# matthewscottgordon/vanrijn

Hardware: AMD Instinct MI355X
Metric: Msamples/s + achieved HBM GB/s, 1024x1024 bunny @256spp, 1/2/4/8 GPUs (higher is better)
Workload: dtype f64; 1 GPU; main.rs scene (plane, 3 spheres, Lambertian bunny), 1024x1024 @256spp per frame split over 1 GPU(s) (256 each); config=c3, width=1024, height=1024, spp_per_gpu=256, triangles=69312, bvh_depth=20, parallelism=spp-split x1, RCCL reduce, streams=1, pmc_key=main 1024x1024 spp256

## Files before the change

include/vanrijn_amd.h:

```cpp
#ifndef VANRIJN_AMD_H
#define VANRIJN_AMD_H

#include <stddef.h>
#include <stdint.h>

#ifdef __cplusplus
extern "C" {
#endif

#define VR_ABI_VERSION 10
#define VR_HAS_FILM 1
#define VR_HAS_ONE_BVH 1
#define VR_MAX_SPECTRUM_SAMPLES 64
#define VR_RECURSION_LIMIT 128

typedef enum vr_status {
    VR_OK = 0,
    VR_ERROR_INVALID_ARGUMENT = -1,
    VR_ERROR_OUT_OF_MEMORY = -2,
    VR_ERROR_DEVICE = -3,
    VR_ERROR_NO_DEVICE = -4,
    VR_ERROR_SINGULAR_BASIS = -5,
    VR_ERROR_IO = -6,
    VR_ERROR_UNSUPPORTED = -7,
// ... 339 lines not shown
void vr_colour_xyz_for_wavelength(double wavelength, double out[3]);
int vr_load_obj(const char* path, uint64_t* triangle_count, double** vertices, double** normals);
void vr_mesh_free(double* vertices, double* normals);
int vr_load_obj_groups(const char* path, uint64_t* triangle_count, double** vertices, double** normals,
                       uint32_t** group, uint32_t* group_count, char** names);
void vr_obj_groups_free(uint32_t* group, char* names);

int vr_tone_map_device(const double* state, uint64_t pixel_count, uint8_t* rgb_out, int device, void* stream);
int vr_tone_map(const double* colour_xyz, uint64_t pixel_count, uint8_t* rgb_out, int device);
int vr_write_png(const char* path, const uint8_t* rgb, uint32_t width, uint32_t height);

int vr_scene_set_staging_limit(vr_scene* scene, uint64_t bytes);

int vr_debug_set_fault_object(vr_scene* scene, int32_t object);

int vr_debug_set_launch_flags(vr_scene* scene, uint32_t flags);
int vr_scene_needs_wide_offsets(uint64_t triangle_count, uint64_t wide_node_count);
#define VR_CHOICE_COUNTING 1u
#define VR_CHOICE_RECORD 2u
#define VR_CHOICE_WHITTED 4u
#define VR_CHOICE_COOP_GATED 8u
#define VR_CHOICE_WIDE_OFFSETS 16u
#define VR_CHOICE_MULTI_BVH 32u
int vr_launch_takes_one_bvh(uint64_t bvh_count, int32_t root4, uint32_t other, int32_t stack_depth, int32_t stack16);
int vr_scene_launch_variant(const vr_scene* scene, uint64_t pixel_samples, uint32_t launch_flags, int32_t recording,
                            uint32_t* variant);

int vr_device_count(void);
const char* vr_last_error(void);
uint32_t vr_abi_version(void);

#ifdef __cplusplus
}
#endif
#endif
```

vanrijn_amd/_native.py:

```python
import ctypes as C
import os

HERE = os.path.dirname(os.path.abspath(__file__))
LIB_PATH = os.environ.get("VR_LIBRARY") or os.path.join(HERE, "lib", "libvanrijn_amd.so")

VR_OK = 0
STATUS = {
    0: "VR_OK", -1: "VR_ERROR_INVALID_ARGUMENT", -2: "VR_ERROR_OUT_OF_MEMORY", -3: "VR_ERROR_DEVICE",
    -4: "VR_ERROR_NO_DEVICE", -5: "VR_ERROR_SINGULAR_BASIS", -6: "VR_ERROR_IO", -7: "VR_ERROR_UNSUPPORTED",
    -8: "VR_ERROR_HOST_ONLY",
}
MATERIAL_LAMBERTIAN, MATERIAL_REFLECTIVE, MATERIAL_PHONG, MATERIAL_DIELECTRIC = 0, 1, 2, 3
PRIMITIVE_PLANE, PRIMITIVE_SPHERE = 0, 1
OBJECT_PRIMITIVE_LIST, OBJECT_BVH = 0, 1
SCENE_HOST_ONLY = 1
SCENE_DEVICE_BVH = 2
SCENE_REFERENCE_BVH = 4
SCENE_DEVICE_SAH = 8
SCENE_GREEDY_COLLAPSE = 16
SCENE_WIDE_OFFSETS = 32
LAUNCH_TIMED, LAUNCH_COUNTERS, LAUNCH_DEFER_TIMES, LAUNCH_NO_CULL = 1, 2, 4, 8
LAUNCH_NO_DIST_CULL, LAUNCH_NO_COOP, LAUNCH_NO_LONE_WALK, LAUNCH_STACK32, LAUNCH_MULTI_BVH = 16, 32, 64, 128, 256
VARIANT_COOP, VARIANT_WIDE_OFFSETS, VARIANT_STACK16, VARIANT_ONE_BVH = 1, 2, 4, 8
CHOICE_COUNTING, CHOICE_RECORD, CHOICE_WHITTED, CHOICE_COOP_GATED, CHOICE_WIDE_OFFSETS, CHOICE_MULTI_BVH = 1, 2, 4, 8, 16, 32
SCENE_INFO_NAN_FREE = 1


class VrError(RuntimeError):
    def __init__(self, code, message):
        super().__init__(f"{STATUS.get(code, code)}: {message}")
        self.code = code


class Vec3(C.Structure):
    _fields_ = [("x", C.c_double), ("y", C.c_double), ("z", C.c_double)]


class CameraPose(C.Structure):
    _fields_ = [("location", Vec3), ("right", Vec3), ("up", Vec3), ("forward", Vec3), ("film_distance", C.c_double)]


class CameraLens(C.Structure):
    _fields_ = [("lens_radius", C.c_double), ("focus_distance", C.c_double)]


class Spectrum(C.Structure):
    _fields_ = [("shortest_wavelength", C.c_double), ("longest_wavelength", C.c_double),
# ... 171 lines not shown
                              C.POINTER(C.POINTER(C.c_double))]),
    "vr_mesh_free": (None, [C.POINTER(C.c_double), C.POINTER(C.c_double)]),
    "vr_load_obj_groups": (C.c_int, [C.c_char_p, C.POINTER(C.c_uint64), C.POINTER(C.POINTER(C.c_double)),
                                     C.POINTER(C.POINTER(C.c_double)), C.POINTER(C.POINTER(C.c_uint32)),
                                     C.POINTER(C.c_uint32), C.POINTER(C.c_void_p)]),
    "vr_obj_groups_free": (None, [C.POINTER(C.c_uint32), C.c_void_p]),
    "vr_tone_map_device": (C.c_int, [_p, _u64, _p, _i32, _p]),
    "vr_tone_map": (C.c_int, [_p, _u64, _p, _i32]),
    "vr_write_png": (C.c_int, [C.c_char_p, _p, _u32, _u32]),
    "vr_film_create": (C.c_int, [_u64, _u64, _i32, C.POINTER(C.c_void_p)]),
    "vr_film_destroy": (None, [_p]),
    "vr_film_clear": (C.c_int, [_p]),
    "vr_film_partial_render_scene": (C.c_int, [_p, _p, TileC, C.POINTER(FilmMerge)]),
    "vr_film_render_tile": (C.c_int, [_p, _p, C.POINTER(RenderParams), C.POINTER(FilmMerge)]),
    "vr_film_merge_state": (C.c_int, [_p, TileC, _p, _p, C.POINTER(FilmMerge)]),
    "vr_film_read": (C.c_int, [_p, C.POINTER(AccumulationBufferC), C.POINTER(C.c_uint64)]),
    "vr_film_to_image_rgb_u8": (C.c_int, [_p, _p, C.POINTER(C.c_uint64)]),
    "vr_film_to_image_rgb_u8_device": (C.c_int, [_p, _p, _p, C.POINTER(C.c_uint64)]),
    "vr_scene_set_staging_limit": (C.c_int, [_p, _u64]),
    "vr_debug_set_fault_object": (C.c_int, [_p, _i32]),
    "vr_debug_set_launch_flags": (C.c_int, [_p, _u32]),
    "vr_scene_needs_wide_offsets": (C.c_int, [_u64, _u64]),
    "vr_launch_takes_one_bvh": (C.c_int, [_u64, C.c_int32, _u32, C.c_int32, C.c_int32]),
    "vr_scene_launch_variant": (C.c_int, [_p, _u64, _u32, C.c_int32, C.POINTER(_u32)]),
    "vr_device_count": (C.c_int, []),
    "vr_last_error": (C.c_char_p, []),
    "vr_abi_version": (C.c_uint32, []),
}

_lib = None


def lib():
    global _lib
    if _lib is None:
        if not os.path.exists(LIB_PATH):
            raise ImportError(f"{LIB_PATH} is missing: run `python -m vanrijn_amd.build` (hipcc, gfx950) first")
        try:
            import torch
        except ImportError:
            pass
        L = C.CDLL(LIB_PATH)
        for name, (res, args) in SIGNATURES.items():
            try:
                fn = getattr(L, name)
            except AttributeError:
# ... 14 lines not shown
```

vanrijn_amd/csrc/vr_device.h:

```cpp
#pragma once

#include <hip/hip_runtime.h>
#include <stdint.h>

#include "../../include/vanrijn_amd.h"
#include "rgb_spectrum_tables.h"
#include "vr_layout.h"

namespace vr {
namespace dev {

struct V3 {
    double x, y, z;
};
__device__ __forceinline__ V3 mk(double x, double y, double z) { return V3{x, y, z}; }
__device__ __forceinline__ V3 add(V3 a, V3 b) { return mk(a.x + b.x, a.y + b.y, a.z + b.z); }
__device__ __forceinline__ V3 sub(V3 a, V3 b) { return mk(a.x - b.x, a.y - b.y, a.z - b.z); }
__device__ __forceinline__ V3 scl(V3 a, double s) { return mk(a.x * s, a.y * s, a.z * s); }
__device__ __forceinline__ V3 neg(V3 a) { return mk(-a.x, -a.y, -a.z); }
__device__ __forceinline__ double dot(V3 a, V3 b) {
    double s = -0.0;
    s = s + a.x * b.x;
    s = s + a.y * b.y;
    s = s + a.z * b.z;
// ... 75 lines not shown
    double after = (double)(i + 1) / (double)(n - 1) * range + shortest;
    double delta = after - before;
    double ratio = (wl - before) / delta;
    return sample(i) * (1.0 - ratio) + sample(i + 1) * ratio;
}

__device__ __forceinline__ double material_colour(const Material* m, double wl) {
    return spectrum_at(m->shortest, m->longest, m->n, wl, [&](int j) { return m->samples[j]; });
}

template <class F>
__device__ __forceinline__ double spectrum_fast(const Material* m, double wl, F sample) {
    if (wl < m->shortest || wl > m->longest) return 0.0;
    const int n = m->n;
    int i = (int)((wl - m->shortest) * m->inv_step);
    i = i < 0 ? 0 : (i > n - 1 ? n - 1 : i);
    if (i == n - 1) return sample(i);
    const double before = m->knots[i], after = m->knots[i + 1];
    const double ratio = (wl - before) / (after - before);
    return sample(i) * (1.0 - ratio) + sample(i + 1) * ratio;
}
__device__ __forceinline__ double material_intensity(const Material* m, double wl) {
    return spectrum_fast(m, wl, [&](int j) { return m->samples[j]; });
}

constexpr double kPi = 3.14159265358979323846;

__device__ __forceinline__ V3 cosine_weighted_hemisphere(Rng& rng) {
    const double ux = rng.open01();
    const double uy = rng.open01();
    const double ox = -1.0 + ux * 2.0, oy = -1.0 + uy * 2.0;
    double px = ox, py = oy;
    if (!(ox == 0.0 && oy == 0.0)) {
        double radius, angle;
        if (fabs(ox) > fabs(oy)) {
            radius = ox;
            angle = ((kPi / 4.0) * oy) / ox;
        } else {
            radius = oy;
            angle = kPi / 2.0 - ((kPi / 4.0) * ox) / oy;
        }
        px = cos(angle) * radius;
        py = sin(angle) * radius;
    }
    const double z = sqrt(fmax(0.0, 1.0 - px * px - py * py));
    return mk(px, py, z);
// ... 22 lines not shown
    } else {
        f.R = 1.0;
        f.T = 0.0;
        f.tdir = mk(0.0, 0.0, 0.0);
    }
    if (w_i.z < 0.0) {
        f.rdir.z *= -1.0;
        f.tdir.z *= -1.0;
    }
    return f;
}
__device__ __forceinline__ Fresnel dielectric_fresnel(const Material* m, V3 w_i, double wl) {
    const double eta = material_colour(m, wl);
    return w_i.z >= 0.0 ? fresnel(w_i, 1.0, eta) : fresnel(w_i, eta, 1.0);
}
__device__ __forceinline__ double dielectric_strength(const Fresnel& f, V3 w_o) {
    const V3 dr = sub(w_o, f.rdir);
    if (dot(dr, dr) < 0.0000000001) return f.R;
    const V3 dt = sub(w_o, f.tdir);
    if (dot(dt, dt) < 0.0000000001) return f.T;
    return 0.0;
}

__device__ double sky_intensity(double wy, double wl, const Material* knots) {
    const double r = wy, g = wy, b = 1.0;
    double c0, c1, c2;
    int kx, ky;
    if (r <= g && r <= b) {
        if (g <= b) { c0 = r; c1 = g - r; c2 = b - g; kx = VR_RGBSPEC_CYAN; ky = VR_RGBSPEC_BLUE; }
        else { c0 = r; c1 = b - r; c2 = g - b; kx = VR_RGBSPEC_CYAN; ky = VR_RGBSPEC_GREEN; }
    } else if (g <= r && g < b) {
        if (r <= b) { c0 = g; c1 = r - g; c2 = b - r; kx = VR_RGBSPEC_MAGENTA; ky = VR_RGBSPEC_BLUE; }
        else { c0 = g; c1 = b - g; c2 = r - b; kx = VR_RGBSPEC_MAGENTA; ky = VR_RGBSPEC_RED; }
    } else {
        if (r <= g) { c0 = b; c1 = r - b; c2 = g - r; kx = VR_RGBSPEC_YELLOW; ky = VR_RGBSPEC_GREEN; }
        else { c0 = b; c1 = g - b; c2 = r - g; kx = VR_RGBSPEC_YELLOW; ky = VR_RGBSPEC_RED; }
    }
    return spectrum_fast(knots, wl, [&](int j) {
        return c0 * c_rgbspec[VR_RGBSPEC_WHITE][j] + c1 * c_rgbspec[kx][j] + c2 * c_rgbspec[ky][j];
    });
}

__device__ __forceinline__ double gaussian(double wl, double alpha, double mu, double s1, double s2) {
    double s = wl < mu ? s1 : s2;
    double denominator = 2.0 * (s * s);
    double t = wl - mu;
    return alpha * exp(-(t * t) / denominator);
}
__device__ __forceinline__ double gaussian_kt(double wl, double alpha, double mu, double k1, double k2,
                                              const double* tab) {
    const double k = wl < mu ? k1 : k2;
    const double t = wl - mu;
    return alpha * vr_exp_tab_near(-(t * t) * k, tab);
}
#define VR_GT(alpha, mu, s1, s2) \
    gaussian_kt(wl, alpha, mu, 1.0 / (2.0 * ((s1) * (s1))), 1.0 / (2.0 * ((s2) * (s2))), tab)
constexpr double kLobeReach = 20000.0;
template <bool ANY_WL>
__device__ __forceinline__ V3 xyz_for_wavelength_tab(double wl, const double* tab) {
    if (ANY_WL) wl = fabs(wl) > kLobeReach ? copysign(kLobeReach, wl) : wl;
    return mk(VR_GT(1.056, 599.8, 37.9, 31.0) + VR_GT(0.362, 442.0, 16.0, 26.7) + VR_GT(-0.065, 501.1, 20.4, 26.2),
              VR_GT(0.821, 568.8, 46.9, 40.5) + VR_GT(0.286, 530.9, 16.3, 31.1),
              VR_GT(1.217, 437.0, 11.8, 36.0) + VR_GT(0.681, 459.0, 26.0, 13.8));
// ... 549 lines not shown
```

vanrijn_amd/csrc/vr_host.cpp:

```cpp
#include "vr_host.h"

#include <chrono>

using namespace vrh;

#ifndef VR_COOP_SAMPLES
#define VR_COOP_SAMPLES (4ull << 20)
#endif
#ifndef VR_COOP_BOUNCES
#define VR_COOP_BOUNCES 0u
#endif
namespace {

static bool needs_big_offsets(uint64_t tri_count, uint64_t wide_count) {
    return tri_count * sizeof(vr::TriVerts) >= (1ull << 32) || wide_count >= (1ull << 25);
}

static bool takes_one_bvh(uint64_t bvh_count, int32_t root4, uint32_t other, int stack_depth, bool s16) {
    if (bvh_count != 1 || root4 < 0 || other != 0) return false;
    return s16 ? stack_depth <= 32 : (stack_depth > 24 && stack_depth <= 32);
}

static bool coop_gated(const vr_scene* s, uint64_t pixel_samples) {
    return pixel_samples <= VR_COOP_SAMPLES && (s->mats & 2) && s->dark0;
}

static vr::LaunchChoice launch_choice(const vr_scene* s, bool coop, bool gated, bool counting, bool recording,
                                      uint32_t launch_flags) {
    vr::LaunchChoice lc;
    const int stack = s->dev.integrator == 1 ? std::max(stack_depth(s), wide_stack_depth(s)) : wide_stack_depth(s);
    lc.stack_depth = stack;
    lc.counting = counting;
    lc.recording = recording;
    lc.dark0 = s->dark0;
    lc.mats = s->mats ? s->mats : 3;
    lc.big = s->force_big || needs_big_offsets(s->tri_count, s->wide_count);
    lc.coop = coop && !recording && !counting && !lc.big && s->dev.integrator != 1 && s->dark0 && (lc.mats & 2);
    lc.s16 = !recording && !counting && !lc.big && !lc.coop && s->dev.integrator != 1 && s->wide_count < 65536 &&
             stack <= 32 && !(launch_flags & VR_LAUNCH_STACK32);
    const uint32_t other = (counting ? VR_CHOICE_COUNTING : 0u) | (recording ? VR_CHOICE_RECORD : 0u) |
                           (s->dev.integrator == 1 ? VR_CHOICE_WHITTED : 0u) | (gated || lc.coop ? VR_CHOICE_COOP_GATED : 0u) |
                           (lc.big ? VR_CHOICE_WIDE_OFFSETS : 0u) |
                           ((launch_flags & VR_LAUNCH_MULTI_BVH) ? VR_CHOICE_MULTI_BVH : 0u);
    lc.one_bvh = takes_one_bvh(s->bvhs.size(), s->bvhs.empty() ? INT32_MIN : s->bvhs[0].root4, other, stack, lc.s16);
    return lc;
}

static uint32_t variant_bits(const vr::LaunchChoice& lc) {
    return (lc.coop ? VR_VARIANT_COOP : 0u) | (lc.big ? VR_VARIANT_WIDE_OFFSETS : 0u) |
           (lc.s16 ? VR_VARIANT_STACK16 : 0u) | (lc.one_bvh ? VR_VARIANT_ONE_BVH : 0u);
}

int grid_per_cu() {
    const char* g = tuning_env("VR_GRID_PER_CU");
    return g ? std::max(1, atoi(g)) : 3;
}
int coop_grid_per_cu() {
    const char* g = tuning_env("VR_COOP_GRID");
    return g ? std::max(1, atoi(g)) : 3;
}

int ctx_acquire(vr_scene* s, CallCtx** out, const hipStream_t* want = nullptr) {
    {
        std::lock_guard<std::mutex> g(s->ctx_mutex);
        for (size_t i = s->ctx_free.size(); i-- > 0;) {
            if (hipEventQuery(s->ctx_free[i]->done) == hipSuccess) {
// ... 74 lines not shown
uint64_t seed_key_of(uint64_t seed) {
    uint64_t z = seed ^ 0x76616E52696A6E31ull;
    z = (z ^ (z >> 30)) * 0xBF58476D1CE4E5B9ull;
    z = (z ^ (z >> 27)) * 0x94D049BB133111EBull;
    return z ^ (z >> 31);
}

vr::RenderArgs make_args(const vr_scene* s, const vr_render_params* p, double* state) {
    vr::RenderArgs a{};
    a.scene = s->dev;
    a.start_column = p->tile.start_column;
    a.start_row = p->tile.start_row;
    a.tile_width = p->tile.end_column - p->tile.start_column;
    a.tile_height = p->tile.end_row - p->tile.start_row;
    a.width = p->width;
    a.height = p->height;
    a.seed = p->seed;
    a.seed_key = seed_key_of(p->seed);
    a.first_sample = p->first_sample;
    a.spp = p->spp;
    a.accumulate = p->accumulate;
    a.state = state;
    a.fault_object = s->fault_object;
    const char* th = tuning_env("VR_SHADE_THRESHOLD");
    a.shade_threshold = th ? (uint32_t)atoi(th) : 52u;
    const char* sm = tuning_env("VR_SHADE_MIN");
    a.shade_min = sm ? (uint32_t)std::max(0, atoi(sm)) : 16u;
    a.early_stop = s->nan_free ? 1u : 0u;
    if (const char* es = tuning_env("VR_EARLY_STOP")) a.early_stop = atoi(es) != 0 && s->nan_free;
    const char* mm = tuning_env("VR_MISS_MIN");
    a.miss_min = mm ? (uint32_t)std::max(0, atoi(mm)) : 8u;
    const char* ch = tuning_env("VR_CHUNK");
    a.chunk = ch ? (uint32_t)std::max(1, atoi(ch)) : 1u;
    const char* ts = tuning_env("VR_TAIL_SAMPLES");
    a.tail_samples = ts ? (uint32_t)std::max(0, atoi(ts)) : 0u;
    const char* gr = tuning_env("VR_GRAB");
    if (gr) {
        a.grab = (uint32_t)std::max(0, atoi(gr));
    } else {
        const uint64_t items = ((a.tile_width + 7) / 8) * ((a.tile_height + 7) / 8) * 64 * std::max(1u, p->spp);
        const uint64_t waves = (uint64_t)std::max(1, s->cu_count) * 3 * 4;
        const uint64_t g = items / (waves * 80) / 64 * 64;
        a.grab = (uint32_t)std::min<uint64_t>(512, std::max<uint64_t>(128, g));
    }
    const char* lt = tuning_env("VR_LEAF_THRESHOLD");
    a.leaf_threshold = lt ? (uint32_t)std::max(1, atoi(lt)) : 48u;
// ... 253 lines not shown
    if (begun_) (void)hipEventRecord(c->done, st);
    if (c) ctx_release(scene_, c);
}

}

template <class T>
static int sum_pass_times(const std::vector<hipEvent_t>& ev, T* kernel_ms, T* reduce_ms) {
    if (!ev.empty()) VR_HIP(hipEventSynchronize(ev.back()));
    for (size_t i = 0; i + 3 <= ev.size(); i += 3) {
        float x = 0.f, y = 0.f;
        VR_HIP(hipEventElapsedTime(&x, ev[i], ev[i + 1]));
        VR_HIP(hipEventElapsedTime(&y, ev[i + 1], ev[i + 2]));
        *kernel_ms += x;
        *reduce_ms += y;
    }
    return VR_OK;
}

int vr_scene_needs_wide_offsets(uint64_t triangle_count, uint64_t wide_node_count) {
    return needs_big_offsets(triangle_count, wide_node_count) ? 1 : 0;
}

int vr_launch_takes_one_bvh(uint64_t bvh_count, int32_t root4, uint32_t other, int32_t stack_depth, int32_t stack16) {
    return takes_one_bvh(bvh_count, root4, other, stack_depth, stack16 != 0) ? 1 : 0;
}

int vr_scene_launch_variant(const vr_scene* s, uint64_t pixel_samples, uint32_t launch_flags, int32_t recording,
                            uint32_t* variant) {
    if (!s || !variant) return fail(VR_ERROR_INVALID_ARGUMENT, "null argument");
    const bool counting = (launch_flags & VR_LAUNCH_COUNTERS) != 0;
    launch_flags |= s->debug_launch_flags;
    const bool gated = coop_gated(s, pixel_samples);
    *variant = variant_bits(launch_choice(s, gated && !(launch_flags & VR_LAUNCH_NO_COOP), gated, counting, recording != 0,
                                          launch_flags));
    return VR_OK;
}

int vr_render_tile_device(const vr_scene* s, const vr_render_params* p, double* state, void* stream,
                          uint32_t launch_flags, vr_launch_stats* stats) {
    int rc = check_render_params(s, p);
    if (rc) return rc;
    if (!state) return fail(VR_ERROR_INVALID_ARGUMENT, "null state");
    VR_HIP(hipSetDevice(s->device));
    hipStream_t st = (hipStream_t)stream;
    vr_scene* ms = const_cast<vr_scene*>(s);
// ... 265 lines not shown
```

vanrijn_amd/csrc/vr_host.h:

```cpp
#pragma once
#include <algorithm>
#include <cmath>
#include <cstdio>
#include <cstdlib>
#include <cstring>
#include <functional>
#include <string>
#include <vector>

#include "../../include/vanrijn_amd.h"
#include "vr_layout.h"

#pragma GCC visibility push(hidden)
namespace vrh {

int fail(int code, const std::string& msg);

inline const char* tuning_env(const char* name) {
#ifdef VR_TUNING_VARIANTS
    return getenv(name);
#else
    (void)name;
    return nullptr;
#endif
// ... 83 lines not shown
    void* d_block = nullptr;
    size_t device_bytes = 0;
    vr::DeviceScene dev{};
    unsigned long long* d_counters = nullptr;
    std::mutex counter_mutex;
    std::atomic<uint64_t> pass_counter{0};
    std::mutex ctx_mutex;
    std::vector<struct CallCtx*> ctx_all, ctx_free;
    std::mutex slot_mutex;
    std::unordered_map<void*, int32_t*> stream_slots;
    struct Deferred {
        std::vector<hipEvent_t> ev;
        std::vector<uint32_t> passes;
    };
    std::unordered_map<void*, Deferred> deferred;
    int cu_count = 0;
    uint64_t partial_seed = 0x5EED0001ull;
    int32_t fault_object = -1;
    uint32_t debug_launch_flags = 0;
    double base_extent = 0.0;
    std::vector<double> mesh_extent;
    std::vector<uint8_t> mesh_finite;
    bool dark0_materials = true;
    std::vector<int> mesh_object;
    std::vector<int> mesh_bvh;
    std::vector<uint32_t> mesh_material;
    std::vector<int32_t> mesh_node_base;
    std::vector<int32_t> mesh_root4;
    bool host_stale = false;
    struct UpdatePlan {
        bool built = false;
        std::vector<uint32_t> slot_src;
        std::vector<int32_t> items2, items4;
        std::vector<uint32_t> first2, first4;
        void* d_plan = nullptr;
        size_t plan_bytes = 0;
        unsigned long long* d_valid = nullptr;
        uint32_t* d_slot_src = nullptr;
        int32_t *d_items2 = nullptr, *d_items4 = nullptr;
        void* d_stage = nullptr;
        size_t stage_bytes = 0;
    };
    std::vector<UpdatePlan> plans;
    uint32_t desc_materials = 0;
    std::vector<std::vector<uint32_t>> prim_rows;
    struct MeshBase {
// ... 35 lines not shown
        if (ptr) (void)hipFree(ptr);
        if (stream) (void)hipStreamDestroy(stream);
    }
};

inline int device_fail(int e, const char* what) {
    return fail(VR_ERROR_DEVICE, std::string(what) + ": " + hipGetErrorString((hipError_t)e));
}
inline int launch_status(int lr) {
    return fail(lr == -1000 ? VR_ERROR_UNSUPPORTED : VR_ERROR_DEVICE, vr::device_error_string(lr));
}
inline int host_only_error() { return fail(VR_ERROR_HOST_ONLY, "scene was created with VR_SCENE_HOST_ONLY"); }
int error_status(int32_t bits);

inline int stack_depth(const vr_scene* s) { return std::max(1, s->max_depth - 1); }
inline int wide_stack_depth(const vr_scene* s) { return s->wide_stack + 1; }

const char* material_row(const vr_material_desc& m, vr::Material& dm);
const char* light_rows(const vr_integrator_desc& ig, std::vector<vr::Material>& rows, std::vector<double>& dirs);
const char* prim_row(const vr_primitive_desc& p, int32_t object, int32_t position, vr::Prim& dp);
void update_base_extent(vr_scene* s);
void update_material_scalars(vr_scene* s);
void update_scalars(vr_scene* s);

void ctx_free_all(CallCtx* c);
int ctx_grow(void** ptr, size_t* have, size_t need, hipEvent_t done);
int ctx_grow_pinned(CallCtx* c, size_t need);
int stream_slot(vr_scene* s, void* stream, int32_t** out);
int read_and_clear_error(int32_t* slot, hipStream_t stream);
int check_render_params(const vr_scene* s, const vr_render_params* p);
uint64_t seed_key_of(uint64_t seed);
vr::RenderArgs make_args(const vr_scene* s, const vr_render_params* p, double* state);
struct PassEvents;
int enqueue_passes(vr_scene* s, CallCtx* c, const vr_render_params* p, double* state, hipStream_t st, int32_t* err,
                   bool counting, bool recording, void* records, unsigned long long* counters,
                   unsigned long long* wg_times, PassEvents* timing = nullptr, uint32_t launch_flags = 0,
                   uint32_t* variant = nullptr);

struct HostCall {
    CallCtx* c = nullptr;
    hipStream_t st = nullptr;
    int begin(const vr_scene* s);
    ~HostCall();
    size_t part(size_t bytes) { return std::exchange(total_, total_ + ((bytes + 255) & ~size_t(255))); }
    int grow() { return ctx_grow(&c->scratch, &c->scratch_bytes, total_, c->done); }
    char* at(size_t offset) const { return (char*)c->scratch + offset; }
// ... 11 lines not shown
```

vanrijn_amd/csrc/vr_host_edit.cpp:

```cpp
#include "vr_host.h"
#include "vr_refit.h"

using namespace vrh;

namespace {

int build_update_plan(vr_scene* s, uint32_t mi) {
    vr_scene::UpdatePlan& p = s->plans[mi];
    if (p.built) return VR_OK;
    const uint64_t n = s->leaf_order[mi].size(), interior = n ? n - 1 : 0;
    const int64_t tri_base = s->mesh_tri_base[mi], node_base = s->mesh_node_base[mi];
    const bool readback = !s->host_only && s->device_bvh;
    std::vector<vr::TriVerts> tv;
    std::vector<vr::Node> bn;
    std::vector<vr::Node4> wn;
    if (readback) {
        tv.resize(n);
        bn.resize(interior);
        wn.resize(s->wide_count);
        VR_HIP(hipMemcpy(tv.data(), s->dev.tris + tri_base, n * sizeof(vr::TriVerts), hipMemcpyDeviceToHost));
        if (interior)
            VR_HIP(hipMemcpy(bn.data(), s->dev.nodes + node_base, interior * sizeof(vr::Node), hipMemcpyDeviceToHost));
        if (s->wide_count)
            VR_HIP(hipMemcpy(wn.data(), s->dev.nodes4, s->wide_count * sizeof(vr::Node4), hipMemcpyDeviceToHost));
// ... 388 lines not shown
            return fail(VR_ERROR_INVALID_ARGUMENT, "scene edit: primitive material out of range");
    }
    uint32_t lo = UINT32_MAX, hi = 0;
    for (uint32_t k = 0; k < count; ++k)
        for (uint32_t row : s->prim_rows[first + k]) {
            const vr::Prim old = s->prims[row];
            (void)prim_row(prims[k], old.object, old.position, s->prims[row]);
            lo = std::min(lo, row);
            hi = std::max(hi, row);
        }
    update_base_extent(s);
    update_scalars(s);
    if (lo > hi) return VR_OK;
    return copy_rows(s, s->dev.prims, sizeof(vr::Prim), lo, &s->prims[lo], (size_t)(hi - lo + 1));
}

int vr_scene_update_material(vr_scene* s, uint32_t index, const vr_material_desc* material) {
    if (!s || !material) return fail(VR_ERROR_INVALID_ARGUMENT, "null scene or material");
    if (index >= s->desc_materials) return fail(VR_ERROR_INVALID_ARGUMENT, "scene edit: material index out of range");
    vr::Material row;
    if (const char* why = material_row(*material, row)) return fail(VR_ERROR_INVALID_ARGUMENT, why);
    s->materials[index] = row;
    update_material_scalars(s);
    update_scalars(s);
    return copy_rows(s, s->dev.materials, sizeof(vr::Material), index, &s->materials[index], 1);
}

int vr_scene_set_lights(vr_scene* s, const vr_integrator_desc* integrator) {
    if (!s) return fail(VR_ERROR_INVALID_ARGUMENT, "null scene");
    const int32_t kind = integrator ? integrator->kind : (int32_t)VR_INTEGRATOR_SIMPLE_RANDOM;
    if (kind != s->dev.integrator || (integrator && (int64_t)integrator->light_count != s->dev.light_count))
        return fail(VR_ERROR_INVALID_ARGUMENT, "scene edit: integrator kind or light_count differs from the scene's");
    if (kind != VR_INTEGRATOR_WHITTED) return VR_OK;
    std::vector<vr::Material> rows;
    std::vector<double> dirs;
    if (const char* why = light_rows(*integrator, rows, dirs)) return fail(VR_ERROR_INVALID_ARGUMENT, why);
    std::copy(rows.begin(), rows.end(), s->materials.begin() + s->dev.light_base);
    s->light_dirs = dirs;
    const int rc = copy_rows(s, s->dev.materials, sizeof(vr::Material), (size_t)s->dev.light_base, rows.data(), rows.size());
    return rc ? rc : copy_rows(s, s->dev.light_dirs, sizeof(double), 0, dirs.data(), dirs.size());
}

int vr_scene_transform_mesh(vr_scene* s, uint32_t mesh, const double matrix[12], void* stream) {
    if (!s || !matrix) return fail(VR_ERROR_INVALID_ARGUMENT, "null scene or matrix");
    if (mesh >= s->leaf_order.size()) return fail(VR_ERROR_INVALID_ARGUMENT, "scene transform: bad mesh index");
    for (int i = 0; i < 12; ++i)
        if (!std::isfinite(matrix[i]))
            return fail(VR_ERROR_INVALID_ARGUMENT, "scene transform: a matrix entry is not finite");
    const uint64_t n = s->leaf_order[mesh].size();
    if (n == 0) return VR_OK;
    const vr::refit::Affine a = affine_of(matrix);
    if (s->host_only) return transform_mesh_host(s, mesh, n, a);
    return transform_mesh_device(s, mesh, n, a, (hipStream_t)stream);
}


namespace {

const char* kMaterialRange = "mesh materials: a material index is out of range";

// ... 89 lines not shown
```

vanrijn_amd/csrc/vr_host_scene.cpp:

```cpp
#include "vr_host.h"

#include "rgb_spectrum_tables.h"

using namespace vrh;

namespace {

struct H3 {
    double x, y, z;
};
double hdot(H3 a, H3 b) {
    double s = -0.0;
    s = s + a.x * b.x;
    s = s + a.y * b.y;
    s = s + a.z * b.z;
    return s;
}
H3 hcross(H3 a, H3 b) { return {a.y * b.z - a.z * b.y, a.z * b.x - a.x * b.z, a.x * b.y - a.y * b.x}; }
H3 hnormalize(H3 a) {
    double inv = 1.0 / std::sqrt(hdot(a, a));
    return {a.x * inv, a.y * inv, a.z * inv};
}

bool shading_finite(const vr_mesh_desc& m) {
// ... 99 lines not shown
void update_base_extent(vr_scene* s) {
    double extent =
        std::max({std::fabs(s->camera[0]), std::fabs(s->camera[1]), std::fabs(s->camera[2])}) + s->lens.lens_radius;
    for (const vr::Prim& p : s->prims) {
        if (p.kind == VR_PRIMITIVE_PLANE)
            extent = std::max(extent, std::fabs(p.scalar));
        else
            extent = std::max({extent, std::fabs(p.vec[0]) + std::fabs(p.scalar), std::fabs(p.vec[1]) + std::fabs(p.scalar),
                               std::fabs(p.vec[2]) + std::fabs(p.scalar)});
    }
    s->base_extent = extent;
}

void update_material_scalars(vr_scene* s) {
    s->mats = 0;
    s->dark0_materials = true;
    for (uint32_t i = 0; i < s->desc_materials; ++i) {
        const vr::Material& m = s->materials[i];
        const vr_spectrum colour{m.shortest, m.longest, (uint32_t)m.n, m.samples};
        if (vr_spectrum_intensity_at_wavelength(&colour, 0.0) != 0.0) s->dark0_materials = false;
        s->mats |= m.kind == VR_MATERIAL_LAMBERTIAN ? 1 : (m.kind == VR_MATERIAL_REFLECTIVE ? 2 : 4);
        if (m.kind == VR_MATERIAL_DIELECTRIC) s->dark0_materials = false;
    }
}

void update_scalars(vr_scene* s) {
    double extent = s->base_extent;
    for (double e : s->mesh_extent) extent = std::max(extent, e);
    s->extent = extent;
    s->dev.margin = 1e-9 * (extent + 1.0);
    s->dev.behind_margin = 1e-6 * (extent + 1.0);
    s->dev.extent = extent;
    s->nan_free = (s->mats & 4) == 0;
    for (uint8_t f : s->mesh_finite)
        if (!f) s->nan_free = false;
    s->dark0 = s->dark0_materials && s->nan_free;
}

}

namespace {

void collapse_scene(vr_scene* s, const std::vector<vr::Node>& nodes) {
    WideTree w = collapse_wide(nodes, s->bvhs, s->greedy_collapse);
    s->nodes4 = std::move(w.nodes4);
    for (size_t i = 0; i < s->bvhs.size(); ++i) s->bvhs[i].root4 = w.roots[i];
// ... 154 lines not shown
        if (const char* why = material_row(desc->materials[i], dm)) return bad(why);
        s->materials.push_back(dm);
    }
    s->desc_materials = desc->material_count;
    update_material_scalars(s);
    if (desc->integrator && desc->integrator->kind == VR_INTEGRATOR_WHITTED) {
        const vr_integrator_desc& ig = *desc->integrator;
        s->dev.integrator = VR_INTEGRATOR_WHITTED;
        s->dev.light_base = (int32_t)s->materials.size();
        s->dev.light_count = (int32_t)ig.light_count;
        if (const char* why = light_rows(ig, s->materials, s->light_dirs)) return bad(why);
    } else if (desc->integrator && desc->integrator->kind != VR_INTEGRATOR_SIMPLE_RANDOM) {
        return bad("unknown integrator kind");
    }
    {
        vr::Material sky{};
        sky.n = 32;
        sky.shortest = VR_RGBSPEC_SHORTEST;
        sky.longest = VR_RGBSPEC_LONGEST;
        fill_knots(sky);
        s->dev.sky_row = (int32_t)s->materials.size();
        s->materials.push_back(sky);
    }
    std::vector<int> mesh_object(desc->mesh_count, -1);
    s->prim_rows.resize(desc->primitive_count);
    for (uint32_t oi = 0; oi < desc->object_count; ++oi) {
        const vr_object_desc& o = desc->objects[oi];
        if (o.kind == VR_OBJECT_PRIMITIVE_LIST) {
            if ((uint64_t)o.first + o.count > desc->primitive_count) return bad("primitive list out of range");
            for (uint32_t k = 0; k < o.count; ++k) {
                const vr_primitive_desc& p = desc->primitives[o.first + k];
                if (p.material >= desc->material_count) return bad("primitive material out of range");
                vr::Prim dp;
                if (const char* why = prim_row(p, (int32_t)oi, (int32_t)k, dp)) return bad(why);
                s->prim_rows[o.first + k].push_back((uint32_t)s->prims.size());
                s->prims.push_back(dp);
            }
        } else if (o.kind == VR_OBJECT_BVH) {
            if (o.first >= desc->mesh_count) return bad("BVH object mesh out of range");
            if (mesh_object[o.first] >= 0) return bad("a mesh can back only one BVH object");
            mesh_object[o.first] = (int)oi;
        } else {
            return bad("unknown object kind");
        }
    }
    s->object_count = desc->object_count;
// ... 254 lines not shown
```

vanrijn_amd/csrc/vr_layout.h:

```cpp
#pragma once

#include <stddef.h>
#include <stdint.h>

namespace vr {

constexpr int kRecursionLimit = 128;
constexpr int kPathCut = 8;
constexpr int kMaxSpectrumSamples = 64;
constexpr double kBounceBias = 0.0000001;
constexpr uint32_t kMaxDeferredLaunches = 4096;

struct alignas(128) Node {
    double box[2][6];
    int32_t child[2];
    int32_t pad[6];
};
static_assert(sizeof(Node) == 128, "Node must be one 128-B line");

constexpr int32_t kEmptyChild = INT32_MIN;
struct alignas(128) Node4 {
    float bound[6][4];
    int32_t child[4];
    int32_t pad[4];
// ... 97 lines not shown
    uint32_t leaf_stall;
    uint32_t leaf_few;
    uint32_t coop;
    uint32_t coop_bounces;
    uint32_t lone_walk;
    uint32_t sort_mask;
    uint32_t item_order;
    int32_t fault_object;
    uint32_t shade_min;
    uint32_t miss_min;
    uint32_t early_stop;
    double film[4];
    double rcp_blocks, rcp_bw;
    unsigned long long* queue;
    double* staging;
    double* state;
    void* records;
    unsigned long long* counters;
    unsigned long long* wg_times;
    int32_t* error_flag;
    const uint8_t* block_mask;
    const uint32_t* live_blocks;
    const uint32_t* live_count;
    uint64_t reserved[4];
    uint32_t* stage_tag;
    uint32_t stage_gen;
    uint32_t posed;
};
static_assert(offsetof(RenderArgs, posed) == 460, "RenderArgs: a member moved");
static_assert(sizeof(RenderArgs) == 464, "RenderArgs: its size changed");

struct TraceArgs {
    DeviceScene scene;
    uint64_t n;
    const double* origins;
    const double* directions;
    void* out;
};

struct QueryArgs {
    DeviceScene scene;
    uint64_t n;
    const double* origins;
    const double* directions;
    void* hits;
    void* records;
    uint32_t flags;
// ... 106 lines not shown
```

vanrijn_amd/csrc/vr_render.hip:

```cpp
#include <hip/hip_runtime.h>

#include <float.h>
#include <stdint.h>
#include <stdlib.h>
#include <type_traits>

#include "../../include/vanrijn_amd.h"
#include "rgb_spectrum_tables.h"
#include "vr_layout.h"
#include "vr_exp_table.h"
#include "vr_camera.h"

#include "vr_device.h"

namespace vr {
namespace dev {

__device__ __forceinline__ Ray ray_new(V3 o, V3 d) { return Ray{o, normalize(d)}; }

__device__ __forceinline__ uint64_t lanes_ieq(int a, int b) { return __builtin_amdgcn_sicmp(a, b, 32); }
__device__ __forceinline__ uint64_t lanes_ine(int a, int b) { return __builtin_amdgcn_sicmp(a, b, 33); }
__device__ __forceinline__ uint64_t lanes_igt(int a, int b) { return __builtin_amdgcn_sicmp(a, b, 38); }
__device__ __forceinline__ uint64_t lanes_ige(int a, int b) { return __builtin_amdgcn_sicmp(a, b, 39); }
__device__ __forceinline__ uint64_t lanes_uge(uint32_t a, uint32_t b) { return __builtin_amdgcn_uicmp(a, b, 35); }
// ... 179 lines not shown
    const uint64_t items = render_items(A, per_chunk);
    const uint64_t rounds = chunk_rounds(A);
    const double rcp_R = A.item_order ? 1.0 / (double)(rounds + tail_of(A)) : 0.0;
    const uint32_t bulk = A.spp - tail_of(A);
    const uint64_t npix = A.tile_width * A.tile_height;
    uint32_t px = 0, py = 0, s_end = 0;
    int state = kNeedRay;
    uint32_t s_idx = 0;
    bool coop_on = false;
    uint64_t w_next = 0, w_end = 0;
    Rng rng;
    rng.reset(0);
    RayPre pre;
    Ray32 pre32;
    NodeOrder near_off = {0u, 32u, 64u};
    Best best;
    int node = -1, sp = 0, bvh_i = 0, cur_object = 0;
#define VR_WALKED_OBJECT (ONE ? S.bvhs[0].object : cur_object)
    int np = 0;
    float cull_far = INFINITY, cull_behind = -INFINITY;
    int depth = -1, bounces = 0, flags = 0;
    double lambda = 0.0, T = 1.0, Acc = 0.0, T0 = 1.0, Acc0 = 0.0, b0 = 0.0, wo_y = 0.0;
    double Wa = 0.0, Wb = 0.0;

    auto culled = [&](double tlo, double thi) {
        const double bound = best.kind ? best.d : INFINITY;
        if (tlo > bound + S.margin * (1.0 + fabs(bound))) return true;
        return pre.behind_ok() && thi < -S.behind_margin;
    };
    auto set_cull_far = [&]() {
        const double bound = best.kind ? best.d : INFINITY;
        cull_far = round_away_f32(bound + S.margin * (1.0 + fabs(bound)) + margin_of(pre32));
    };
    auto tri_at = [&](int tri) -> const TriVerts* {
        if (BIG) return VR_TRIS + (uint32_t)tri;
        return (const TriVerts*)((const char*)VR_TRIS + (uint32_t)tri * (uint32_t)sizeof(TriVerts));
    };
    typedef int32_t vr_i4 __attribute__((ext_vector_type(4)));
    auto load_quads = [&](int n, const NodeOrder& no, vr_f4 (&q)[6], int (&c)[4]) {
        const char* const p = BIG ? (const char*)(VR_NODES4 + (uint32_t)n) : (const char*)VR_NODES4;
        const uint32_t b = BIG ? 0u : (uint32_t)n << 7;
        vr_f4 q0 = *(const vr_f4*)(p + (b | no.x)), q1 = *(const vr_f4*)(p + ((b | no.x) ^ 16u));
        vr_f4 q2 = *(const vr_f4*)(p + (b | no.y)), q3 = *(const vr_f4*)(p + ((b | no.y) ^ 16u));
        vr_f4 q4 = *(const vr_f4*)(p + (b | no.z)), q5 = *(const vr_f4*)(p + ((b | no.z) ^ 16u));
        vr_i4 ch = *(const vr_i4*)(p + (size_t)b + 96);
        asm volatile("" : "+v"(q0), "+v"(q1), "+v"(q2), "+v"(q3), "+v"(q4), "+v"(q5), "+v"(ch));
// ... 329 lines not shown
            const V3 inv0 = mk((1.0 * (m11 * m22 - m12 * m21)) * det, (-1.0 * (m01 * m22 - m02 * m21)) * det,
                               (1.0 * (m01 * m12 - m02 * m11)) * det);
            wo_world.x = dot(inv0, w_o);
            const V3 inv1 = mk((-1.0 * (m10 * m22 - m12 * m20)) * det, (1.0 * (m00 * m22 - m02 * m20)) * det,
                               (-1.0 * (m00 * m12 - m02 * m10)) * det);
            wo_world.y = dot(inv1, w_o);
            const V3 inv2 = mk((1.0 * (m10 * m21 - m11 * m20)) * det, (-1.0 * (m00 * m21 - m01 * m20)) * det,
                               (1.0 * (m00 * m11 - m01 * m10)) * det);
            wo_world.z = dot(inv2, w_o);
        }
        const double cosf = fabs(dot(wo_world, h.normal));
        if constexpr (WHITTED) {
            double ba, bb;
            bsdf_affine(mat, w_i, w_o, lambda, ba, bb);
            Wa = (T * ba) * cosf;
            Wb = (T * bb) * cosf;
            const V3 d1 = normalize_n1(wo_world);
            ++bounces;
            pre.o = add(h.loc, scl(d1, kBounceBias));
            pre.d = normalize_n1(d1);
            state = kRayReady;
            return;
        }
        const double c_l = material_intensity(mat, lambda);
        const double c_0 = DARK0 ? 0.0 : material_intensity(mat, 0.0);
        double a, a0, bterm;
        bool cut = false;
        if (kind == 1) {
            if (w_i.z <= 0.0 || w_o.z <= 0.0) {
                a = 0.0; a0 = 0.0; bterm = 0.0; cut = true;
            } else {
                const V3 refl = mk(-w_o.x, -w_o.y, w_o.z);
                double cth = dot(w_i, refl);
                cth = cth < 0.0 ? 0.0 : (cth > 1.0 ? 1.0 : cth);
                const double theta = acos(fabs(cth));
                const double sigma = 0.05, two = 2.0;
                const double f = mat->reflection * exp(-(pow(theta, two)) / (two * sigma * sigma));
                a = (((pdf * cosf) * c_l) * mat->diffuse) * (1.0 - f);
                a0 = (((pdf * cosf) * c_0) * mat->diffuse) * (1.0 - f);
                bterm = f;
            }
        } else if (MATS == 3 && kind == 2) {
            if (w_i.z < 0.0 || w_o.z < 0.0) {
                a = 0.0; a0 = 0.0; bterm = 0.0; cut = true;
            } else {
                const V3 refl = mk(-w_i.x, -w_i.y, w_i.z);
                a = ((pdf * cosf) * c_l) * mat->diffuse;
                a0 = ((pdf * cosf) * c_0) * mat->diffuse;
                bterm = pow(fabs(dot(w_o, refl)), mat->smoothness) * (mat->reflection / dot(w_i, mk(0.0, 0.0, 1.0)));
            }
        } else if (MATS == 3 && kind == 3) {
            a = (pdf * cosf) * dielectric_strength(fr, w_o);
            a0 = DARK0 ? 0.0 : (pdf * cosf) * dielectric_strength(dielectric_fresnel(mat, w_i, 0.0), w_o);
            bterm = 0.0;
        } else {
            a = ((pdf * cosf) * c_l) * mat->diffuse;
            a0 = ((pdf * cosf) * c_0) * mat->diffuse;
            bterm = 0.0;
        }
        if (depth == 0) b0 = bterm;
        if (!(flags & kPathCut)) {
            Acc = Acc + T * bterm;
            T = T * a;
            if (!DARK0) {
                Acc0 = Acc0 + T0 * bterm;
                T0 = T0 * a0;
            }
        }
        if (cut) flags |= kPathCut;
        const bool zero_tail = DARK0 ? (b0 == 0.0) : (T0 == 0.0 && Acc0 == 0.0);
        if (!RECORD && A.early_stop && T == 0.0 && Acc == 0.0 && zero_tail) {
            finish(lambda, 0.0);
            return;
        }
        wo_y = wo_world.y;
        const V3 d1 = normalize_n1(wo_world);
        ++bounces;
        pre.o = add(h.loc, scl(d1, kBounceBias));
        pre.d = normalize_n1(d1);
        state = kRayReady;
    };

    auto coop_vaddr = [&](int o, uint32_t om, int v) {
        const int j = v / STACK, og = (int)(om & 3) - 1, op = (int)(om >> 8);
        int col;
        if (j == 0) {
            col = o;
        } else if (og < 0) {
            col = (o + j) & 63;
        } else {
            const int s1 = o < op ? o : op, s2 = o < op ? op : o, lo = og * 32;
            col = lo + j - 1;
// ... 281 lines not shown
                const uint64_t done_trav = lanes_ieq(state, kTraversed);
                const int nhit = __popcll(done_trav & lanes_ine((int)best.kind, (int)kNone));
                const int nmiss = __popcll(done_trav & lanes_ieq((int)best.kind, (int)kNone));
                shade_now = nhit >= (int)A.shade_min || idle;
                finish_now = nmiss >= (int)A.miss_min || idle;
            }
            if (state == kTraversed && (best.kind == kNone ? finish_now : shade_now)) {
                VR_MARK("traversed");
                bool go = false;
                fin = false;
                if (WHITTED && depth >= 0) {
                    if (!best.kind) {
                        finish(lambda, Acc);
                    } else {
                        Acc = Acc + Wb;
                        T = Wa;
                        depth += 1;
                        go = true;
                    }
                } else if (depth < 0) {
                    if (!best.kind) {
                        finish(0.0, 0.0);
                    } else {
                        flags |= 1;
                        lambda = 380.0 + (740.0 - 380.0) * rng.standard();
                        T = 1.0; Acc = 0.0; T0 = 1.0; Acc0 = 0.0; b0 = 0.0;
                        depth = 0;
                        go = true;
                    }
                } else if (!best.kind) {
                    finish(lambda, (flags & kPathCut) ? Acc : Acc + T * sky_intensity(wo_y, lambda, &S.materials[S.sky_row]));
                } else {
                    depth += 1;
                    if (depth == kRecursionLimit) {
                        flags |= 2;
                        finish(0.0, DARK0 ? b0 : (flags & kPathCut) ? Acc0 : Acc0 + T0 * 0.0);
                    } else {
                        go = true;
                    }
                }
                if (go) shade();
                if (fin) store_photon(fin_wl, fin_I);
            }
            VR_STAMP(0);
            VR_MARK("refill_check");
            while (true) {
                const bool need = state == kNeedRay && s_idx >= s_end;
                const uint64_t m = lanes_ieq(state, kNeedRay) & lanes_uge(s_idx, s_end);
                if (m == 0) break;
                VR_SEC(7);
                VR_MARK("refill");
                const unsigned leader = (unsigned)__builtin_ctzll(m);
                const uint32_t rank = (uint32_t)lanes_below(m);
                unsigned long long base = 0;
                bool take = need;
                if (A.grab == 0) {
                    if (lane == leader) base = atomicAdd(A.queue, (unsigned long long)__popcll(m));
                    base = __shfl(base, (int)leader);
                } else {
// ... 786 lines not shown
```

vanrijn_amd/scene.py:

```python
from dataclasses import dataclass, field
import atexit
import ctypes as C
from enum import Enum
from typing import List
import weakref

import numpy as np

from . import _native as N

_LIVE = weakref.WeakSet()


@atexit.register
def _release_live_scenes():
    for s in list(_LIVE):
        s.release()

SHORTEST_VISIBLE_WAVELENGTH = 380.0
LONGEST_VISIBLE_WAVELENGTH = 740.0


class NamedColour(Enum):
    Black = (0.0, 0.0, 0.0)
# ... 415 lines not shown
        if h:
            self.handle = None
            self._destroy(h)

    def __del__(self):
        self.release()

    def set_staging_limit(self, nbytes):
        N.check(N.lib().vr_scene_set_staging_limit(self.handle, int(nbytes)))

    def info(self):
        i = N.SceneInfo()
        N.check(N.lib().vr_scene_get_info(self.handle, C.byref(i)))
        d = {n: getattr(i, n) for n, _ in i._fields_}
        d["nan_free"] = bool(d["flags"] & N.SCENE_INFO_NAN_FREE)
        return d

    def launch_variant(self, pixel_samples, launch_flags=0, recording=False):
        v = C.c_uint32(0)
        N.check(N.lib().vr_scene_launch_variant(self.handle, int(pixel_samples), int(launch_flags), int(bool(recording)),
                                                C.byref(v)))
        return v.value

    def set_fault_object(self, obj):
        N.check(N.lib().vr_debug_set_fault_object(self.handle, obj))

    def set_launch_flags(self, no_cull=False, no_dist_cull=False, no_coop=False, no_lone_walk=False, stack32=False,
                         multi_bvh=False):
        flags = ((N.LAUNCH_NO_CULL if no_cull else 0) | (N.LAUNCH_NO_DIST_CULL if no_dist_cull else 0) |
                 (N.LAUNCH_NO_COOP if no_coop else 0) | (N.LAUNCH_NO_LONE_WALK if no_lone_walk else 0) |
                 (N.LAUNCH_STACK32 if stack32 else 0) | (N.LAUNCH_MULTI_BVH if multi_bvh else 0))
        N.check(N.lib().vr_debug_set_launch_flags(self.handle, flags))

    NODE_DTYPE = np.dtype([("box", "<f8", (2, 6)), ("child", "<i4", (2,)), ("pad", "<i4", (6,))])

    def bvh_nodes(self):
        out = np.zeros(self.info()["node_count"], dtype=self.NODE_DTYPE)
        if out.size:
            N.check(N.lib().vr_scene_bvh_nodes(self.handle, out.ctypes.data_as(C.c_void_p)))
        return out

    def leaf_order(self, mesh):
        out = np.zeros(len(self.spec.meshes[mesh].vertices), dtype=np.uint64)
        N.check(N.lib().vr_scene_bvh_leaf_order(self.handle, mesh, out.ctypes.data_as(C.c_void_p)))
        return out

# ... 131 lines not shown
```

Baseline: 7481 Msamples/s.

## Carry per-path wavelength segment across bounces when material spectrum grids are shared

Detects on the host when all material rows (and optionally the sky) use identical wavelength knot grids. When they do, the device computes the spectrum segment index and interpolation ratio once per path, at wavelength sampling time, and reuses it for every bounce's material and sky lookup instead of re-searching the knots each time. For Lambertian-only dark scenes it also drops path-cut flag bookkeeping. A launch-choice bit is added so a separate specialization is selected, which adds register pressure for the carried segment and more kernel variants.

```diff
diff --git a/include/vanrijn_amd.h b/include/vanrijn_amd.h
--- a/include/vanrijn_amd.h
+++ b/include/vanrijn_amd.h
@@ -385,7 +385,10 @@
 #define VR_CHOICE_COOP_GATED 8u
 #define VR_CHOICE_WIDE_OFFSETS 16u
 #define VR_CHOICE_MULTI_BVH 32u
+#define VR_CHOICE_OWN_GRIDS 64u
 int vr_launch_takes_one_bvh(uint64_t bvh_count, int32_t root4, uint32_t other, int32_t stack_depth, int32_t stack16);
+int vr_material_grids_shared(const void* rows, uint32_t count);
+int vr_scene_grid_shared(const vr_scene* scene);
 int vr_scene_launch_variant(const vr_scene* scene, uint64_t pixel_samples, uint32_t launch_flags, int32_t recording,
                             uint32_t* variant);
 
diff --git a/vanrijn_amd/_native.py b/vanrijn_amd/_native.py
--- a/vanrijn_amd/_native.py
+++ b/vanrijn_amd/_native.py
@@ -23,6 +23,7 @@
 LAUNCH_NO_DIST_CULL, LAUNCH_NO_COOP, LAUNCH_NO_LONE_WALK, LAUNCH_STACK32, LAUNCH_MULTI_BVH = 16, 32, 64, 128, 256
 VARIANT_COOP, VARIANT_WIDE_OFFSETS, VARIANT_STACK16, VARIANT_ONE_BVH = 1, 2, 4, 8
 CHOICE_COUNTING, CHOICE_RECORD, CHOICE_WHITTED, CHOICE_COOP_GATED, CHOICE_WIDE_OFFSETS, CHOICE_MULTI_BVH = 1, 2, 4, 8, 16, 32
+CHOICE_OWN_GRIDS = 64
 SCENE_INFO_NAN_FREE = 1
 
 
@@ -240,6 +241,8 @@
     "vr_debug_set_launch_flags": (C.c_int, [_p, _u32]),
     "vr_scene_needs_wide_offsets": (C.c_int, [_u64, _u64]),
     "vr_launch_takes_one_bvh": (C.c_int, [_u64, C.c_int32, _u32, C.c_int32, C.c_int32]),
+    "vr_material_grids_shared": (C.c_int, [_p, _u32]),
+    "vr_scene_grid_shared": (C.c_int, [_p]),
     "vr_scene_launch_variant": (C.c_int, [_p, _u64, _u32, C.c_int32, C.POINTER(_u32)]),
     "vr_device_count": (C.c_int, []),
     "vr_last_error": (C.c_char_p, []),
diff --git a/vanrijn_amd/csrc/vr_device.h b/vanrijn_amd/csrc/vr_device.h
--- a/vanrijn_amd/csrc/vr_device.h
+++ b/vanrijn_amd/csrc/vr_device.h
@@ -121,6 +121,31 @@
 }
 __device__ __forceinline__ double material_intensity(const Material* m, double wl) {
     return spectrum_fast(m, wl, [&](int j) { return m->samples[j]; });
+}
+
+__device__ __forceinline__ void path_segment(const Material* g, double wl, int& seg, double& ratio) {
+    seg = -1;
+    ratio = 0.0;
+    if (wl < g->shortest || wl > g->longest) return;
+    const int n = g->n;
+    int i = (int)((wl - g->shortest) * g->inv_step);
+    i = i < 0 ? 0 : (i > n - 1 ? n - 1 : i);
+    seg = i;
+    if (i == n - 1) return;
+    const double before = g->knots[i], after = g->knots[i + 1];
+    ratio = (wl - before) / (after - before);
+}
+template <class F>
+__device__ __forceinline__ double spectrum_path(const Material* g, int seg, double ratio, F sample) {
+    if (seg < 0) return 0.0;
+    if (seg == g->n - 1) return sample(seg);
+    return sample(seg) * (1.0 - ratio) + sample(seg + 1) * ratio;
+}
+__device__ __forceinline__ double material_intensity_on(const Material* m, const Material* g, double wl) {
+    return spectrum_fast(g, wl, [&](int j) { return m->samples[j]; });
+}
+__device__ __forceinline__ double material_intensity_path(const Material* m, const Material* g, int seg, double ratio) {
+    return spectrum_path(g, seg, ratio, [&](int j) { return m->samples[j]; });
 }
 
 constexpr double kPi = 3.14159265358979323846;
@@ -189,7 +214,8 @@
     return 0.0;
 }
 
-__device__ double sky_intensity(double wy, double wl, const Material* knots) {
+template <class L>
+__device__ __forceinline__ double sky_spectrum(double wy, L lookup) {
     const double r = wy, g = wy, b = 1.0;
     double c0, c1, c2;
     int kx, ky;
@@ -203,9 +229,15 @@
         if (r <= g) { c0 = b; c1 = r - b; c2 = g - r; kx = VR_RGBSPEC_YELLOW; ky = VR_RGBSPEC_GREEN; }
         else { c0 = b; c1 = g - b; c2 = r - g; kx = VR_RGBSPEC_YELLOW; ky = VR_RGBSPEC_RED; }
     }
-    return spectrum_fast(knots, wl, [&](int j) {
+    return lookup([&](int j) {
         return c0 * c_rgbspec[VR_RGBSPEC_WHITE][j] + c1 * c_rgbspec[kx][j] + c2 * c_rgbspec[ky][j];
     });
+}
+__device__ double sky_intensity(double wy, double wl, const Material* knots) {
+    return sky_spectrum(wy, [&](auto sample) { return spectrum_fast(knots, wl, sample); });
+}
+__device__ double sky_intensity_path(double wy, const Material* g, int seg, double ratio) {
+    return sky_spectrum(wy, [&](auto sample) { return spectrum_path(g, seg, ratio, sample); });
 }
 
 __device__ __forceinline__ double gaussian(double wl, double alpha, double mu, double s1, double s2) {
diff --git a/vanrijn_amd/csrc/vr_host.cpp b/vanrijn_amd/csrc/vr_host.cpp
--- a/vanrijn_amd/csrc/vr_host.cpp
+++ b/vanrijn_amd/csrc/vr_host.cpp
@@ -41,7 +41,8 @@
     const uint32_t other = (counting ? VR_CHOICE_COUNTING : 0u) | (recording ? VR_CHOICE_RECORD : 0u) |
                            (s->dev.integrator == 1 ? VR_CHOICE_WHITTED : 0u) | (gated || lc.coop ? VR_CHOICE_COOP_GATED : 0u) |
                            (lc.big ? VR_CHOICE_WIDE_OFFSETS : 0u) |
-                           ((launch_flags & VR_LAUNCH_MULTI_BVH) ? VR_CHOICE_MULTI_BVH : 0u);
+                           ((launch_flags & VR_LAUNCH_MULTI_BVH) ? VR_CHOICE_MULTI_BVH : 0u) |
+                           (lc.dark0 && (lc.mats == 1 || lc.mats == 2) && !s->grid_shared ? VR_CHOICE_OWN_GRIDS : 0u);
     lc.one_bvh = takes_one_bvh(s->bvhs.size(), s->bvhs.empty() ? INT32_MIN : s->bvhs[0].root4, other, stack, lc.s16);
     return lc;
 }
@@ -162,6 +163,7 @@
     a.accumulate = p->accumulate;
     a.state = state;
     a.fault_object = s->fault_object;
+    a.sky_on_grid = s->sky_on_grid ? 1u : 0u;
     const char* th = tuning_env("VR_SHADE_THRESHOLD");
     a.shade_threshold = th ? (uint32_t)atoi(th) : 52u;
     const char* sm = tuning_env("VR_SHADE_MIN");
@@ -461,6 +463,12 @@
     return needs_big_offsets(triangle_count, wide_node_count) ? 1 : 0;
 }
 
+int vr_material_grids_shared(const void* rows, uint32_t count) {
+    return rows && grids_shared((const vr::Material*)rows, count) ? 1 : 0;
+}
+
+int vr_scene_grid_shared(const vr_scene* s) { return s ? (s->grid_shared ? 1 : 0) | (s->sky_on_grid ? 2 : 0) : 0; }
+
 int vr_launch_takes_one_bvh(uint64_t bvh_count, int32_t root4, uint32_t other, int32_t stack_depth, int32_t stack16) {
     return takes_one_bvh(bvh_count, root4, other, stack_depth, stack16 != 0) ? 1 : 0;
 }
diff --git a/vanrijn_amd/csrc/vr_host.h b/vanrijn_amd/csrc/vr_host.h
--- a/vanrijn_amd/csrc/vr_host.h
+++ b/vanrijn_amd/csrc/vr_host.h
@@ -129,6 +129,7 @@
     std::vector<double> mesh_extent;
     std::vector<uint8_t> mesh_finite;
     bool dark0_materials = true;
+    bool grid_shared = false, sky_on_grid = false;
     std::vector<int> mesh_object;
     std::vector<int> mesh_bvh;
     std::vector<uint32_t> mesh_material;
@@ -210,6 +211,8 @@
 void update_base_extent(vr_scene* s);
 void update_material_scalars(vr_scene* s);
 void update_scalars(vr_scene* s);
+bool grids_shared(const vr::Material* rows, size_t count);
+void update_grid_shared(vr_scene* s);
 
 void ctx_free_all(CallCtx* c);
 int ctx_grow(void** ptr, size_t* have, size_t need, hipEvent_t done);
diff --git a/vanrijn_amd/csrc/vr_host_edit.cpp b/vanrijn_amd/csrc/vr_host_edit.cpp
--- a/vanrijn_amd/csrc/vr_host_edit.cpp
+++ b/vanrijn_amd/csrc/vr_host_edit.cpp
@@ -434,6 +434,7 @@
     if (const char* why = material_row(*material, row)) return fail(VR_ERROR_INVALID_ARGUMENT, why);
     s->materials[index] = row;
     update_material_scalars(s);
+    update_grid_shared(s);
     update_scalars(s);
     return copy_rows(s, s->dev.materials, sizeof(vr::Material), index, &s->materials[index], 1);
 }
@@ -448,6 +449,7 @@
     std::vector<double> dirs;
     if (const char* why = light_rows(*integrator, rows, dirs)) return fail(VR_ERROR_INVALID_ARGUMENT, why);
     std::copy(rows.begin(), rows.end(), s->materials.begin() + s->dev.light_base);
+    update_grid_shared(s);
     s->light_dirs = dirs;
     const int rc = copy_rows(s, s->dev.materials, sizeof(vr::Material), (size_t)s->dev.light_base, rows.data(), rows.size());
     return rc ? rc : copy_rows(s, s->dev.light_dirs, sizeof(double), 0, dirs.data(), dirs.size());
diff --git a/vanrijn_amd/csrc/vr_host_scene.cpp b/vanrijn_amd/csrc/vr_host_scene.cpp
--- a/vanrijn_amd/csrc/vr_host_scene.cpp
+++ b/vanrijn_amd/csrc/vr_host_scene.cpp
@@ -145,6 +145,23 @@
         s->mats |= m.kind == VR_MATERIAL_LAMBERTIAN ? 1 : (m.kind == VR_MATERIAL_REFLECTIVE ? 2 : 4);
         if (m.kind == VR_MATERIAL_DIELECTRIC) s->dark0_materials = false;
     }
+}
+
+bool grids_shared(const vr::Material* rows, size_t count) {
+    for (size_t i = 1; i < count; ++i) {
+        const vr::Material &a = rows[0], &b = rows[i];
+        if (a.n != b.n || a.n < 0 || a.n > vr::kMaxSpectrumSamples) return false;
+        if (std::memcmp(&a.shortest, &b.shortest, sizeof(double)) || std::memcmp(&a.longest, &b.longest, sizeof(double)) ||
+            std::memcmp(&a.inv_step, &b.inv_step, sizeof(double)) ||
+            std::memcmp(a.knots, b.knots, sizeof(double) * (size_t)a.n))
+            return false;
+    }
+    return true;
+}
+
+void update_grid_shared(vr_scene* s) {
+    s->grid_shared = grids_shared(s->materials.data(), (size_t)s->dev.sky_row);
+    s->sky_on_grid = s->grid_shared && grids_shared(s->materials.data(), s->materials.size());
 }
 
 void update_scalars(vr_scene* s) {
@@ -345,6 +362,7 @@
         s->dev.sky_row = (int32_t)s->materials.size();
         s->materials.push_back(sky);
     }
+    update_grid_shared(s);
     std::vector<int> mesh_object(desc->mesh_count, -1);
     s->prim_rows.resize(desc->primitive_count);
     for (uint32_t oi = 0; oi < desc->object_count; ++oi) {
diff --git a/vanrijn_amd/csrc/vr_layout.h b/vanrijn_amd/csrc/vr_layout.h
--- a/vanrijn_amd/csrc/vr_layout.h
+++ b/vanrijn_amd/csrc/vr_layout.h
@@ -143,7 +143,9 @@
     const uint8_t* block_mask;
     const uint32_t* live_blocks;
     const uint32_t* live_count;
-    uint64_t reserved[4];
+    uint32_t sky_on_grid;
+    uint32_t reserved32;
+    uint64_t reserved[3];
     uint32_t* stage_tag;
     uint32_t stage_gen;
     uint32_t posed;
diff --git a/vanrijn_amd/csrc/vr_render.hip b/vanrijn_amd/csrc/vr_render.hip
--- a/vanrijn_amd/csrc/vr_render.hip
+++ b/vanrijn_amd/csrc/vr_render.hip
@@ -225,6 +225,12 @@
     int depth = -1, bounces = 0, flags = 0;
     double lambda = 0.0, T = 1.0, Acc = 0.0, T0 = 1.0, Acc0 = 0.0, b0 = 0.0, wo_y = 0.0;
     double Wa = 0.0, Wb = 0.0;
+    constexpr bool PATHWL = ONE && DARK0 && (MATS == 1 || MATS == 2) && !WHITTED && !COUNT && !RECORD;
+    constexpr bool CARRY = PATHWL && MATS == 1, NOFLAGS = CARRY;
+#define VR_PATH_CUT (!NOFLAGS && (flags & kPathCut))
+    const Material* const grid = S.materials;
+    int wl_seg = -1;
+    double wl_ratio = 0.0;
 
     auto culled = [&](double tlo, double thi) {
         const double bound = best.kind ? best.d : INFINITY;
@@ -600,7 +606,9 @@
             state = kRayReady;
             return;
         }
-        const double c_l = material_intensity(mat, lambda);
+        const double c_l = CARRY    ? material_intensity_path(mat, grid, wl_seg, wl_ratio)
+                           : PATHWL ? material_intensity_on(mat, grid, lambda)
+                                    : material_intensity(mat, lambda);
         const double c_0 = DARK0 ? 0.0 : material_intensity(mat, 0.0);
         double a, a0, bterm;
         bool cut = false;
@@ -637,7 +645,7 @@
             bterm = 0.0;
         }
         if (depth == 0) b0 = bterm;
-        if (!(flags & kPathCut)) {
+        if (!VR_PATH_CUT) {
             Acc = Acc + T * bterm;
             T = T * a;
             if (!DARK0) {
@@ -645,7 +653,7 @@
                 T0 = T0 * a0;
             }
         }
-        if (cut) flags |= kPathCut;
+        if (!NOFLAGS && cut) flags |= kPathCut;
         const bool zero_tail = DARK0 ? (b0 == 0.0) : (T0 == 0.0 && Acc0 == 0.0);
         if (!RECORD && A.early_stop && T == 0.0 && Acc == 0.0 && zero_tail) {
             finish(lambda, 0.0);
@@ -973,19 +981,22 @@
                     if (!best.kind) {
                         finish(0.0, 0.0);
                     } else {
-                        flags |= 1;
+                        if (!NOFLAGS) flags |= 1;
                         lambda = 380.0 + (740.0 - 380.0) * rng.standard();
+                        if constexpr (CARRY) path_segment(grid, lambda, wl_seg, wl_ratio);
                         T = 1.0; Acc = 0.0; T0 = 1.0; Acc0 = 0.0; b0 = 0.0;
                         depth = 0;
                         go = true;
                     }
                 } else if (!best.kind) {
-                    finish(lambda, (flags & kPathCut) ? Acc : Acc + T * sky_intensity(wo_y, lambda, &S.materials[S.sky_row]));
+                    finish(lambda, VR_PATH_CUT              ? Acc
+                                   : CARRY && A.sky_on_grid ? Acc + T * sky_intensity_path(wo_y, grid, wl_seg, wl_ratio)
+                                                            : Acc + T * sky_intensity(wo_y, lambda, &S.materials[S.sky_row]));
                 } else {
                     depth += 1;
                     if (depth == kRecursionLimit) {
-                        flags |= 2;
-                        finish(0.0, DARK0 ? b0 : (flags & kPathCut) ? Acc0 : Acc0 + T0 * 0.0);
+                        if (!NOFLAGS) flags |= 2;
+                        finish(0.0, DARK0 ? b0 : VR_PATH_CUT ? Acc0 : Acc0 + T0 * 0.0);
                     } else {
                         go = true;
                     }
diff --git a/vanrijn_amd/scene.py b/vanrijn_amd/scene.py
--- a/vanrijn_amd/scene.py
+++ b/vanrijn_amd/scene.py
@@ -461,6 +461,14 @@
                                                 C.byref(v)))
         return v.value
 
+    def grid_shared(self):
+        return int(N.lib().vr_scene_grid_shared(self.handle))
+
+    @classmethod
+    def grids_shared(cls, rows):
+        rows = np.ascontiguousarray(rows, dtype=cls.MATERIAL_DTYPE)
+        return bool(N.lib().vr_material_grids_shared(rows.ctypes.data_as(C.c_void_p), len(rows)))
+
     def set_fault_object(self, obj):
         N.check(N.lib().vr_debug_set_fault_object(self.handle, obj))
 
```

Result: faster. 7582 Msamples/s (median of 6 runs) (+1.3%).
